# ilyakurdyukov/jpeg-quantsmooth

Measured on AMD Instinct MI355X. Metric: 8x8 blocks/s at q=3 niter=3, higher is better.
Workload: dtype f32

## Files before the change

### jpeg-quantsmooth_amd/csrc/qs_devfn.h

```cpp
#pragma once
#include <hip/hip_runtime.h>
#include <stdint.h>
#include "qs_device.h"

__device__ __forceinline__ int f2i_x86(float v) {
  return (v >= -2147483648.0f && v < 2147483648.0f) ? (int)v : (int)0x80000000;
}

__device__ __forceinline__ float round_half_away(float x) {
  float t = __builtin_truncf(x);
  float fr = __builtin_fabsf(x - t);
  return fr >= 0.5f ? t + __builtin_copysignf(1.0f, x) : t;
}

__device__ __forceinline__ void interval(int c, int div, int x1, int sh, int& orig, int& lo, int& hi) {
  int a = ((x1 * c) >> 16) + c;
  a = (int)(((uint32_t)a << sh) + 0x4000u) >> 15;
  a *= div;
  const int d0 = (div - 1) >> 1, d1 = div >> 1;
  orig = a;
  hi = a + (a < 0 ? d1 : d0);
  lo = a - (a > 0 ? d1 : d0);
}


__device__ __forceinline__ int qs_set_find(const QsPlaneSet& set, int w) {
  int lo = 0, hi = set.n - 1;
  while (lo < hi) {
    const int mid = (lo + hi + 1) >> 1;
    if (set.wave0[mid] <= w) lo = mid; else hi = mid - 1;
  }
  return lo;
}
```

### jpeg-quantsmooth_amd/csrc/qs_device.h

```cpp
#pragma once
#include <stdint.h>

#define QS_APRON_X 16
#define QS_LDS_PITCH 65
#define QS_TAB_MAX 272

enum {
  QS_DIAGONALS = 1, QS_JOINT_YUV = 2, QS_UPSAMPLE_UV = 4, QS_LOW_QUALITY = 8,
  QS_NO_REBALANCE = 16, QS_NO_REBALANCE_UV = 32, QS_TRANSCODE = 64
};

struct QsConsts {
  int32_t nat[64];
  int32_t q[64];
  int32_t qraw[64];
  int32_t x1[64];
  int32_t x2[64];
  float   range[64];
  int32_t qn[64], x1n[64], x2n[64];
  int32_t tab_size;
  int32_t pad[15];
  float   tab[64 * QS_TAB_MAX];
  int32_t rec[64][4];
};
enum {
  QS_REC_H_ANY = 1,
  QS_REC_H_SKIP4 = 2,
  QS_REC_H_EVEN = 4,
  QS_REC_V_ANY = 8,
  QS_REC_V_SKIP4 = 16,
  QS_REC_V_EVEN = 32,
  QS_REC_LDS_SHIFT = 6,
  QS_REC_NXT_SHIFT = 12,
  QS_REC_Q1 = 1 << 21
};

static inline int qs_plane_pitch(int wblk) {
  return ((wblk * 8 + QS_APRON_X + 1) + 63) & ~63;
}

#define QS_MAX_PLANES 56
struct QsPlaneRef {
  const QsConsts* cst;
  int16_t* coef;
  uint8_t* plane;
  int32_t* status;
  int32_t wblk, hblk, pitch;
  int32_t mode;
  uint8_t* plane_next;
};
enum {
  QS_PLANE_REBALANCE = 1,
  QS_PLANE_REP_TOP = 2,
  QS_PLANE_REP_BOT = 4
};
struct QsPlaneAux {
  const uint8_t* p[QS_MAX_PLANES];
};
struct QsPlaneSet {
  int32_t n, pad;
  int32_t wave0[QS_MAX_PLANES + 2];
  QsPlaneRef ref[QS_MAX_PLANES];
};
```

### jpeg-quantsmooth_amd/csrc/qs_kernels.hip

```cpp
#include <hip/hip_runtime.h>
#include <stdint.h>
#include <stdlib.h>
#include "qs_device.h"



__device__ __forceinline__ void wave_lds_sync() {
  __builtin_amdgcn_fence(__ATOMIC_RELEASE, "wavefront");
  __builtin_amdgcn_wave_barrier();
  __builtin_amdgcn_fence(__ATOMIC_ACQUIRE, "wavefront");
}

__device__ __forceinline__ uint32_t mulc(uint32_t a, int c) {
  return (uint32_t)__mul24((int)a, c);
}

__device__ __forceinline__ uint32_t lshl13_add(uint32_t x, uint32_t b) {
  uint32_t r;
  asm("v_lshl_add_u32 %0, %1, 13, %2" : "=v"(r) : "v"(x), "v"(b));
  return r;
}

__device__ __forceinline__ void idct8(uint32_t (&v)[8], uint32_t bias) {
  uint32_t z1, z2, z3, z4, z5, t0, t1, t2, t3, e0, e1, e2, e3;
  z2 = v[2]; z3 = v[6];
  z1 = mulc(z2 + z3, 4433);
  asm volatile("" : "+v"(z1));
  t2 = z1 - mulc(z3, 15137);
  t3 = z1 + mulc(z2, 6270);
  t0 = lshl13_add(v[0] + v[4], bias);
  t1 = lshl13_add(v[0] - v[4], bias);
  e0 = t0 + t3; e3 = t0 - t3; e1 = t1 + t2; e2 = t1 - t2;
  t0 = v[7]; t1 = v[5]; t2 = v[3]; t3 = v[1];
  z1 = t0 + t3; z2 = t1 + t2; z3 = t0 + t2; z4 = t1 + t3;
  z5 = mulc(z3 + z4, 9633);
  asm volatile("" : "+v"(z5));
  t0 = mulc(t0, 2446);  t1 = mulc(t1, 16819);
  t2 = mulc(t2, 25172); t3 = mulc(t3, 12299);
  z1 = mulc(z1, 7373);  z2 = mulc(z2, 20995);
  z3 = mulc(z3, 16069); z4 = mulc(z4, 3196);
  z3 = z5 - z3; z4 = z5 - z4;
  t0 += z3 - z1; t1 += z4 - z2; t2 += z3 - z2; t3 += z4 - z1;
  v[0] = e0 + t3; v[7] = e0 - t3;
  v[1] = e1 + t2; v[6] = e1 - t2;
  v[2] = e2 + t1; v[5] = e2 - t1;
  v[3] = e3 + t0; v[4] = e3 - t0;
}

__device__ __forceinline__ void idct_pass1(uint32_t (&ws)[64]) {
#pragma unroll
  for (int x = 0; x < 8; ++x) {
    uint32_t col[8];
#pragma unroll
    for (int j = 0; j < 8; ++j) col[j] = ws[j * 8 + x];
    idct8(col, 1024u);
#pragma unroll
    for (int j = 0; j < 8; ++j) ws[j * 8 + x] = (uint32_t)((int32_t)col[j] >> 11);
  }
}

__device__ __forceinline__ void idct_pass2_row(uint32_t (&row)[8], int (&out)[8]) {
  idct8(row, 257u << 17);
#pragma unroll
  for (int j = 0; j < 8; ++j) {
    int z = (int32_t)row[j];
    z = min(max(z, 0), (256 << 18) - 1);
    out[j] = z >> 18;
  }
}

#define QS_PIX_BITS 0x45000000u
__device__ __forceinline__ void idct_pass2_row_f(uint32_t (&row)[8], float (&out)[8]) {
  idct8(row, 257u << 17);
#pragma unroll
  for (int j = 0; j < 8; ++j) {
    int z = (int32_t)row[j];
    z = min(max(z, 0), (256 << 18) - 1);
    out[j] = __builtin_bit_cast(float, __builtin_amdgcn_alignbit(QS_PIX_BITS >> 14, (uint32_t)z, 18));
  }
}
__device__ __forceinline__ float pix_from_byte(uint32_t v, int n) {
  return __builtin_bit_cast(float, QS_PIX_BITS | ((v >> (8 * n)) & 0xffu));
}

__device__ __forceinline__ void
store_pixel_row(uint8_t* __restrict__ org, int pitch, int y, const int (&o)[8], int bx, int by, int wblk, int hblk,
                int rep_top, int rep_bot) {
  uint2 pk;
  pk.x = (uint32_t)o[0] | ((uint32_t)o[1] << 8) | ((uint32_t)o[2] << 16) | ((uint32_t)o[3] << 24);
  pk.y = (uint32_t)o[4] | ((uint32_t)o[5] << 8) | ((uint32_t)o[6] << 16) | ((uint32_t)o[7] << 24);
  uint8_t* rp = org + (size_t)y * pitch;
  *reinterpret_cast<uint2*>(rp) = pk;
  const bool top = (y == 0 && by == 0 && rep_top), bot = (y == 7 && by == hblk - 1 && rep_bot);
  if (bx == 0) {
    rp[-1] = (uint8_t)o[0];
    if (top) rp[-1 - pitch] = (uint8_t)o[0];
    if (bot) rp[-1 + pitch] = (uint8_t)o[0];
  }
  if (bx == wblk - 1) {
    rp[8] = (uint8_t)o[7];
    if (top) rp[8 - pitch] = (uint8_t)o[7];
    if (bot) rp[8 + pitch] = (uint8_t)o[7];
  }
  if (top) *reinterpret_cast<uint2*>(rp - pitch) = pk;
  if (bot) *reinterpret_cast<uint2*>(rp + pitch) = pk;
}

__device__ __forceinline__ void
idct_ws_to_plane(uint32_t (&ws)[64], uint8_t* __restrict__ plane, int wblk, int hblk, int pitch,
                 int rep_top, int rep_bot, int blk) {
  const int by = blk / wblk, bx = blk - by * wblk;
  idct_pass1(ws);
  uint8_t* org = plane + (size_t)(by * 8 + 1) * pitch + QS_APRON_X + bx * 8;
#pragma unroll
  for (int y = 0; y < 8; ++y) {
    uint32_t row[8]; int o[8];
#pragma unroll
    for (int j = 0; j < 8; ++j) row[j] = ws[y * 8 + j];
    idct_pass2_row(row, o);
    store_pixel_row(org, pitch, y, o, bx, by, wblk, hblk, rep_top, rep_bot);
  }
}

__device__ __forceinline__ void
idct_block_to_plane(const QsConsts* __restrict__ cst, int16_t* __restrict__ coef,
                    uint8_t* __restrict__ plane, int wblk, int hblk, int pitch,
                    int first, int rep_top, int rep_bot, int* __restrict__ status, int blk) {
  uint4* cp = reinterpret_cast<uint4*>(coef) + (size_t)blk * 8;
  uint32_t ws[64];
#pragma unroll
  for (int j = 0; j < 8; ++j) {
    uint4 v = cp[j];
    uint32_t d[4] = {v.x, v.y, v.z, v.w};
#pragma unroll
    for (int c = 0; c < 4; ++c) {
      ws[j * 8 + c * 2] = (uint32_t)(int32_t)(int16_t)(d[c] & 0xffff);
      ws[j * 8 + c * 2 + 1] = (uint32_t)((int32_t)d[c] >> 16);
    }
  }
  if (first) {
    int bad = 0;
#pragma unroll
    for (int j = 0; j < 8; ++j) {
      uint32_t d[4];
#pragma unroll
      for (int c = 0; c < 4; ++c) {
        int lo = (int32_t)ws[j * 8 + c * 2] * cst->qraw[j * 8 + c * 2];
        int hi = (int32_t)ws[j * 8 + c * 2 + 1] * cst->qraw[j * 8 + c * 2 + 1];
        bad |= ((unsigned)(lo + 0x800) > 0xfffu) | ((unsigned)(hi + 0x800) > 0xfffu);
        lo = (int16_t)lo; hi = (int16_t)hi;
        ws[j * 8 + c * 2] = (uint32_t)lo; ws[j * 8 + c * 2 + 1] = (uint32_t)hi;
        d[c] = ((uint32_t)lo & 0xffffu) | ((uint32_t)hi << 16);
      }
      cp[j] = make_uint4(d[0], d[1], d[2], d[3]);
    }
    if (bad) atomicOr(status, 1);
  }
  idct_ws_to_plane(ws, plane, wblk, hblk, pitch, rep_top, rep_bot, blk);
}

__global__ void __launch_bounds__(256)
qs_idct_plane_kernel(const QsConsts* __restrict__ cst, int16_t* __restrict__ coef,
                     uint8_t* __restrict__ plane, int wblk, int hblk, int pitch,
                     int first, int rep_top, int rep_bot, int* __restrict__ status) {
  const int blk = blockIdx.x * 256 + threadIdx.x;
  if (blk >= wblk * hblk) return;
  idct_block_to_plane(cst, coef, plane, wblk, hblk, pitch, first, rep_top, rep_bot, status, blk);
}

#include "qs_devfn.h"

__global__ void __launch_bounds__(256)
qs_idct_set_kernel(const QsPlaneSet set, int first) {
  const int w = __builtin_amdgcn_readfirstlane((int)(blockIdx.x * 4 + (threadIdx.x >> 6)));
  if (w >= set.wave0[set.n]) return;
  const int i = qs_set_find(set, w);
  const QsPlaneRef& r = set.ref[i];
  const int blk = (w - set.wave0[i]) * 64 + (threadIdx.x & 63);
  if (blk >= r.wblk * r.hblk) return;
  idct_block_to_plane(r.cst, r.coef, r.plane, r.wblk, r.hblk, r.pitch, first,
                      r.mode & QS_PLANE_REP_TOP, r.mode & QS_PLANE_REP_BOT, r.status, blk);
}



typedef int16_t __attribute__((may_alias)) lds_i16;
__device__ __forceinline__ int lds_coef(const uint32_t* col, int i) {
  const lds_i16* p = reinterpret_cast<const lds_i16*>(col + (i >> 1) * QS_LDS_PITCH) + (i & 1);
  return *p;
}
__device__ __forceinline__ void lds_set_coef(uint32_t* col, int i, int v) {
  lds_i16* p = reinterpret_cast<lds_i16*>(col + (i >> 1) * QS_LDS_PITCH) + (i & 1);
  *p = (lds_i16)v;
}

static_assert(QS_LDS_PITCH * 4 == 260, "the literal offsets below assume a 260-byte row pitch");
#define QS_LDS16_GROUP(BASE, W, N0) \
  asm volatile("ds_read_i16 %0, %16\n\tds_read_i16 %1, %16 offset:2\n\t" \
               "ds_read_i16 %2, %16 offset:260\n\tds_read_i16 %3, %16 offset:262\n\t" \
               "ds_read_i16 %4, %16 offset:520\n\tds_read_i16 %5, %16 offset:522\n\t" \
               "ds_read_i16 %6, %16 offset:780\n\tds_read_i16 %7, %16 offset:782\n\t" \
               "ds_read_i16 %8, %16 offset:1040\n\tds_read_i16 %9, %16 offset:1042\n\t" \
               "ds_read_i16 %10, %16 offset:1300\n\tds_read_i16 %11, %16 offset:1302\n\t" \
               "ds_read_i16 %12, %16 offset:1560\n\tds_read_i16 %13, %16 offset:1562\n\t" \
               "ds_read_i16 %14, %16 offset:1820\n\tds_read_i16 %15, %16 offset:1822\n\t" \
               "s_waitcnt lgkmcnt(0)" \
               : "=&v"(W[(N0) + 0]), "=&v"(W[(N0) + 1]), "=&v"(W[(N0) + 2]), "=&v"(W[(N0) + 3]), \
                 "=&v"(W[(N0) + 4]), "=&v"(W[(N0) + 5]), "=&v"(W[(N0) + 6]), "=&v"(W[(N0) + 7]), \
                 "=&v"(W[(N0) + 8]), "=&v"(W[(N0) + 9]), "=&v"(W[(N0) + 10]), "=&v"(W[(N0) + 11]), \
                 "=&v"(W[(N0) + 12]), "=&v"(W[(N0) + 13]), "=&v"(W[(N0) + 14]), "=&v"(W[(N0) + 15]) \
               : "v"(BASE) : "memory")
__device__ __forceinline__ void lds_read_block_i16(const uint32_t* col, uint32_t (&ws)[64]) {
  typedef const __attribute__((address_space(3))) uint32_t* lds_ptr;
  const uint32_t a0 = (uint32_t)(uintptr_t)(lds_ptr)col;
  const uint32_t a1 = a0 + 8 * 260, a2 = a0 + 16 * 260, a3 = a0 + 24 * 260;
  QS_LDS16_GROUP(a0, ws, 0);
  QS_LDS16_GROUP(a1, ws, 16);
  QS_LDS16_GROUP(a2, ws, 32);
  QS_LDS16_GROUP(a3, ws, 48);
}

#define QS_PIX_SCALE 0.000244140625f
#define QS_TERM_D(D, W) { \
    float u_ = __builtin_amdgcn_fmed3f(Rs - __builtin_fabsf(D), 0.0f, 1.0f); \
    float t_ = u_ * u_; \
    float x_ = (D) * t_; \
    float y_ = (W) * t_; \
    num = num + x_ * y_; \
    den = den + y_ * y_; }
#define QS_TERM(A, B, W) { float d_ = (A) - (B); QS_TERM_D(d_, W) }

typedef float qs_w16 __attribute__((ext_vector_type(16)));
typedef int qs_i4 __attribute__((ext_vector_type(4)));
#define QS_SWAIT(BUF) asm volatile("s_waitcnt lgkmcnt(0)" : "+s"(BUF) : : "memory")

#define QS_WAVES_PER_WG 4
#define QS_SMOOTH_MIN_WAVES 3
#define QS_RESIDENT_WG (256 * QS_SMOOTH_MIN_WAVES * 4 / QS_WAVES_PER_WG)
#define QS_PRIO_SLOW 3
#define QS_PRIO_TERMS 0

#define QS_TERM_OPT(COND, A, B, W) { float d_, t_; \
        asm volatile( \
          "s_cmp_lg_u32 %[c], 0\n\t" \
          "s_cbranch_scc1 1f\n\t" \
          "v_sub_f32 %[d], %[a], %[b]\n\t" \
          "v_sub_f32 %[t], %[r], |%[d]| clamp\n\t" \
          "v_mul_f32 %[t], %[t], %[t]\n\t" \
          "v_mul_f32 %[d], %[d], %[t]\n\t" \
          "v_mul_f32 %[t], %[w], %[t]\n\t" \
          "v_mul_f32 %[d], %[d], %[t]\n\t" \
          "v_add_f32 %[n], %[n], %[d]\n\t" \
          "v_mul_f32 %[d], %[t], %[t]\n\t" \
          "v_add_f32 %[e], %[e], %[d]\n" \
          "1:" \
          : [n] "+v"(num), [e] "+v"(den), [d] "=&v"(d_), [t] "=&v"(t_) \
          : [a] "v"(A), [b] "v"(B), [w] "s"(W), [r] "s"(Rs), [c] "s"(COND) : "scc"); }
#define QS_TERM_ASM(A, B, W) { float d_, t_; \
        asm volatile( \
          "v_sub_f32 %[d], %[a], %[b]\n\t" \
          "v_sub_f32 %[t], %[r], |%[d]| clamp\n\t" \
          "v_mul_f32 %[t], %[t], %[t]\n\t" \
          "v_mul_f32 %[d], %[d], %[t]\n\t" \
          "v_mul_f32 %[t], %[w], %[t]\n\t" \
          "v_mul_f32 %[d], %[d], %[t]\n\t" \
          "v_add_f32 %[n], %[n], %[d]\n\t" \
          "v_mul_f32 %[d], %[t], %[t]\n\t" \
          "v_add_f32 %[e], %[e], %[d]" \
          : [n] "+v"(num), [e] "+v"(den), [d] "=&v"(d_), [t] "=&v"(t_) \
          : [a] "v"(A), [b] "v"(B), [w] "s"(W), [r] "s"(Rs)); }

#define QS_TERM_D_ASM(D, W) { float d_, t_; \
        asm volatile( \
          "v_sub_f32 %[t], %[r], |%[a]| clamp\n\t" \
          "v_mul_f32 %[t], %[t], %[t]\n\t" \
          "v_mul_f32 %[d], %[a], %[t]\n\t" \
          "v_mul_f32 %[t], %[w], %[t]\n\t" \
          "v_mul_f32 %[d], %[d], %[t]\n\t" \
          "v_add_f32 %[n], %[n], %[d]\n\t" \
          "v_mul_f32 %[d], %[t], %[t]\n\t" \
          "v_add_f32 %[e], %[e], %[d]" \
          : [n] "+v"(num), [e] "+v"(den), [d] "=&v"(d_), [t] "=&v"(t_) \
          : [a] "v"(D), [w] "s"(W), [r] "s"(Rs)); }
#define QS_HOIST 20
#ifndef QS_HOIST_DIAG
#define QS_HOIST_DIAG 32
#endif
#ifndef QS_Q1_SKIP
#define QS_Q1_SKIP 1
#endif
#ifndef QS_STASH
#define QS_STASH 1
#endif

#define QS_SMOOTH_KERNEL_NAME qs_smooth_plane_kernel
#include "qs_smooth_kernel.inc"
#undef QS_SMOOTH_KERNEL_NAME
#define QS_SMOOTH_KERNEL_NAME qs_smooth_set_kernel
#define QS_SMOOTH_SET 1
#include "qs_smooth_kernel.inc"
#undef QS_SMOOTH_KERNEL_NAME
#undef QS_SMOOTH_SET

#define QS_DP_KERNEL_NAME qs_smooth_dp_kernel
#include "qs_smooth_dp_kernel.inc"
#undef QS_DP_KERNEL_NAME
#define QS_DP_KERNEL_NAME qs_smooth_dp_set_kernel
#define QS_DP_SET 1
#include "qs_smooth_dp_kernel.inc"
#undef QS_DP_KERNEL_NAME
#undef QS_DP_SET

__global__ void __launch_bounds__(256)
qs_clamp_kernel(int16_t* __restrict__ coef, size_t nvec) {
  size_t i = (size_t)blockIdx.x * 256 + threadIdx.x;
  const size_t stride = (size_t)gridDim.x * 256;
  uint4* p = reinterpret_cast<uint4*>(coef);
  for (; i < nvec; i += stride) {
    uint4 v = p[i];
    uint32_t d[4] = {v.x, v.y, v.z, v.w};
#pragma unroll
    for (int c = 0; c < 4; ++c) {
      int lo = (int16_t)(d[c] & 0xffff), hi = (int32_t)d[c] >> 16;
      lo = min(max(lo, -1023), 1023); hi = min(max(hi, -1023), 1023);
      d[c] = ((uint32_t)lo & 0xffffu) | ((uint32_t)hi << 16);
    }
    p[i] = make_uint4(d[0], d[1], d[2], d[3]);
  }
}

__global__ void __launch_bounds__(256)
qs_dequant_kernel(const QsConsts* __restrict__ cst, int16_t* __restrict__ coef, size_t nvec) {
  size_t i = (size_t)blockIdx.x * 256 + threadIdx.x;
  const size_t stride = (size_t)gridDim.x * 256;
  uint4* p = reinterpret_cast<uint4*>(coef);
  for (; i < nvec; i += stride) {
    uint4 v = p[i];
    uint32_t d[4] = {v.x, v.y, v.z, v.w};
    const int j = (int)(i & 7);
#pragma unroll
    for (int c = 0; c < 4; ++c) {
      int lo = (int16_t)(d[c] & 0xffff), hi = (int32_t)d[c] >> 16;
      lo *= cst->qraw[j * 8 + c * 2]; hi *= cst->qraw[j * 8 + c * 2 + 1];
      d[c] = ((uint32_t)lo & 0xffffu) | ((uint32_t)hi << 16);
    }
    p[i] = make_uint4(d[0], d[1], d[2], d[3]);
  }
}

#include "qs_launch.h"

void qs_launch_idct_plane(const QsConsts* cst, int16_t* coef, uint8_t* plane, int wblk, int hblk,
                          int first, int rep_top, int rep_bot, int* status, hipStream_t s) {
  const int nblk = wblk * hblk;
  hipLaunchKernelGGL(qs_idct_plane_kernel, dim3((nblk + 255) / 256), dim3(256), 0, s,
                     cst, coef, plane, wblk, hblk, qs_plane_pitch(wblk), first, rep_top, rep_bot, status);
}

#define QS_DP_WAVES 4
static int qs_dp_waves(int groups) {
  static const int on = [] { const char* v = getenv("QS_HIP_DP"); return v ? atoi(v) : 1; }();
  static const int lim = [] { const char* v = getenv("QS_HIP_DP_GROUPS"); return v ? atoi(v) : 768; }();
  static const int lim2 = [] { const char* v = getenv("QS_HIP_DP_GROUPS2"); return v ? atoi(v) : 1536; }();
  if (!on) return 0;
  return groups <= lim ? QS_DP_WAVES : groups <= lim2 ? 2 : 0;
}

void qs_launch_smooth_plane(const QsConsts* cst, int16_t* coef, const uint8_t* plane, uint8_t* plane_next, int rep_top, int rep_bot,
                            int wblk, int hblk, int diag, int rebalance, int final_clamp, int blk_begin, int blk_end, hipStream_t s) {
  const int n = blk_end - blk_begin;
  if (n <= 0) return;
  const int pitch = qs_plane_pitch(wblk);
  const int rep = (rep_top ? QS_PLANE_REP_TOP : 0) | (rep_bot ? QS_PLANE_REP_BOT : 0);
  if (const int nw = qs_dp_waves((n + 63) / 64)) {
    const dim3 g((n + 63) / 64), b(64 * nw);
#define QS_GO_DP(D, W) hipLaunchKernelGGL((qs_smooth_dp_kernel<D, W>), g, b, 0, s, cst, coef, plane, plane_next, rep, wblk, hblk, pitch, rebalance, final_clamp, blk_begin, blk_end)
    if (nw == 2) { if (diag) QS_GO_DP(true, 2); else QS_GO_DP(false, 2); }
    else if (diag) QS_GO_DP(true, QS_DP_WAVES); else QS_GO_DP(false, QS_DP_WAVES);
#undef QS_GO_DP
    return;
  }
  const int per_wg = 64 * QS_WAVES_PER_WG;
  const dim3 grid((n + per_wg - 1) / per_wg), block(per_wg);
#define QS_GO(K) hipLaunchKernelGGL(K, grid, block, 0, s, cst, coef, plane, plane_next, rep, wblk, hblk, pitch, rebalance, final_clamp, blk_begin, blk_end)
  if (diag) QS_GO(qs_smooth_plane_kernel<true>); else QS_GO(qs_smooth_plane_kernel<false>);
#undef QS_GO
}

void qs_launch_idct_set(const QsPlaneSet& set, int first, hipStream_t s) {
  const int nw = set.wave0[set.n];
  if (nw <= 0) return;
  hipLaunchKernelGGL(qs_idct_set_kernel, dim3((nw + 3) / 4), dim3(256), 0, s, set, first);
}

void qs_launch_smooth_set(const QsPlaneSet& set, int diag, int final_clamp, hipStream_t s) {
  const int nw = set.wave0[set.n];
  if (nw <= 0) return;
  if (const int dw = qs_dp_waves(nw)) {
    const dim3 g(nw), b(64 * dw);
#define QS_GO_DP(D, W) hipLaunchKernelGGL((qs_smooth_dp_set_kernel<D, W>), g, b, 0, s, set, final_clamp)
    if (dw == 2) { if (diag) QS_GO_DP(true, 2); else QS_GO_DP(false, 2); }
    else if (diag) QS_GO_DP(true, QS_DP_WAVES); else QS_GO_DP(false, QS_DP_WAVES);
#undef QS_GO_DP
    return;
  }
  const dim3 grid((nw + QS_WAVES_PER_WG - 1) / QS_WAVES_PER_WG), block(64 * QS_WAVES_PER_WG);
  if (diag) hipLaunchKernelGGL(qs_smooth_set_kernel<true>, grid, block, 0, s, set, final_clamp);
  else      hipLaunchKernelGGL(qs_smooth_set_kernel<false>, grid, block, 0, s, set, final_clamp);
}

void qs_launch_clamp(int16_t* coef, size_t nblk, hipStream_t s) {
  const size_t nvec = nblk * 8;
  const int grid = (int)((nvec + 255) / 256 < 8192 ? (nvec + 255) / 256 : 8192);
  hipLaunchKernelGGL(qs_clamp_kernel, dim3(grid ? grid : 1), dim3(256), 0, s, coef, nvec);
}

void qs_launch_dequant(const QsConsts* cst, int16_t* coef, size_t nblk, hipStream_t s) {
  const size_t nvec = nblk * 8;
  const int grid = (int)((nvec + 255) / 256 < 8192 ? (nvec + 255) / 256 : 8192);
  hipLaunchKernelGGL(qs_dequant_kernel, dim3(grid ? grid : 1), dim3(256), 0, s, cst, coef, nvec);
}
```

### jpeg-quantsmooth_amd/csrc/qs_smooth_kernel.inc

```
template <bool DIAG>
__global__ void __launch_bounds__(64 * QS_WAVES_PER_WG, QS_SMOOTH_MIN_WAVES)
#ifdef QS_SMOOTH_SET
QS_SMOOTH_KERNEL_NAME(const QsPlaneSet set, int final_clamp) {
  __shared__ uint32_t lds_all[QS_WAVES_PER_WG][32 * QS_LDS_PITCH];
#if QS_STASH
  __shared__ uint32_t stash_all[QS_WAVES_PER_WG][2 * 8 * 64];
#endif
  const int lane = threadIdx.x & 63, wave = threadIdx.x >> 6;
  uint32_t* lds = lds_all[wave];
  uint32_t* col = lds + lane;
  const int gw = __builtin_amdgcn_readfirstlane((int)(blockIdx.x * QS_WAVES_PER_WG + wave));
  if (gw >= set.wave0[set.n]) return;
  const int pi = qs_set_find(set, gw);
  const QsConsts* __restrict__ cst = set.ref[pi].cst;
  int16_t* __restrict__ coef = set.ref[pi].coef;
  const uint8_t* __restrict__ plane = set.ref[pi].plane;
  const int wblk = set.ref[pi].wblk, hblk = set.ref[pi].hblk, pitch = set.ref[pi].pitch;
  const int rebalance = set.ref[pi].mode & QS_PLANE_REBALANCE;
  const int nblk = wblk * hblk;
  const int base = (gw - set.wave0[pi]) * 64;
  (void)hblk;
#else
QS_SMOOTH_KERNEL_NAME(const QsConsts* __restrict__ cst, int16_t* __restrict__ coef,
                       const uint8_t* __restrict__ plane, uint8_t* __restrict__ plane_next, int rep,
                       int wblk, int hblk, int pitch,
                       int rebalance, int final_clamp, int blk_begin, int blk_end) {
  __shared__ uint32_t lds_all[QS_WAVES_PER_WG][32 * QS_LDS_PITCH];
#if QS_STASH
  __shared__ uint32_t stash_all[QS_WAVES_PER_WG][2 * 8 * 64];
#endif
  const int lane = threadIdx.x & 63, wave = threadIdx.x >> 6;
  uint32_t* lds = lds_all[wave];
  uint32_t* col = lds + lane;
  const int nblk = blk_end;
  const int base = blk_begin + (blockIdx.x * QS_WAVES_PER_WG + wave) * 64;
#endif
  if (base >= nblk) return;
  const int tail_prio = __builtin_amdgcn_readfirstlane(
      (gridDim.x > QS_RESIDENT_WG && blockIdx.x >= (gridDim.x / QS_RESIDENT_WG) * QS_RESIDENT_WG) ? 1 : 0);
  const int nvec = min(64, nblk - base) * 8;
#ifdef QS_STAGGER
  { unsigned hwid; asm volatile("s_getreg_b32 %0, hwreg(HW_REG_HW_ID)" : "=s"(hwid)); if (hwid & 1u) __builtin_amdgcn_s_sleep(QS_STAGGER); }
#endif

  uint4* gsrc = reinterpret_cast<uint4*>(coef) + (size_t)base * 8;
  {
    const int m0 = (lane & 7) * 4;
#pragma unroll
    for (int j = 0; j < 8; ++j) {
      const int idx = j * 64 + lane;
      uint4 v = make_uint4(0, 0, 0, 0);
      if (idx < nvec) v = gsrc[idx];
      uint32_t* dst = lds + m0 * QS_LDS_PITCH + (j * 8 + (lane >> 3));
      dst[0] = v.x; dst[QS_LDS_PITCH] = v.y; dst[2 * QS_LDS_PITCH] = v.z; dst[3 * QS_LDS_PITCH] = v.w;
    }
  }

  const int blk = min(base + lane, nblk - 1);
  const int by = blk / wblk, bx = blk - by * wblk;
  const uint8_t* org = plane + (size_t)(by * 8 + 1) * pitch + QS_APRON_X + bx * 8;
  uint32_t edge[8];
  {
    const uint2 t = *reinterpret_cast<const uint2*>(org - pitch);
    const uint2 b = *reinterpret_cast<const uint2*>(org + (size_t)8 * pitch);
    edge[0] = t.x; edge[1] = t.y; edge[2] = b.x; edge[3] = b.y;
    uint32_t l[8], r[8];
#pragma unroll
    for (int y = 0; y < 8; ++y) {
      l[y] = org[(ptrdiff_t)y * pitch - 1];
      r[y] = org[(ptrdiff_t)y * pitch + 8];
    }
    edge[4] = l[0] | (l[1] << 8) | (l[2] << 16) | (l[3] << 24);
    edge[5] = l[4] | (l[5] << 8) | (l[6] << 16) | (l[7] << 24);
    edge[6] = r[0] | (r[1] << 8) | (r[2] << 16) | (r[3] << 24);
    edge[7] = r[4] | (r[5] << 8) | (r[6] << 16) | (r[7] << 24);
  }
  wave_lds_sync();

  constexpr int TS = DIAG ? 272 : 160;
  float px[64];
  float bd[32];
  constexpr int NH = DIAG ? QS_HOIST_DIAG : QS_HOIST;
  float hd[NH];

  int kfirst = 63;
#if QS_STASH
  int stash_hi = 0;
#endif
  uint32_t chg = 0;
  long long reb_m0 = 0, reb_m1 = 0;
  const float* tabp = cst->tab;
  const int32_t* recp = &cst->rec[0][0];
  qs_w16 WA, WB;
  qs_i4 REC;
  qs_i4 RECN;
  asm volatile("s_load_dwordx4 %0, %2, %3\n\ts_load_dwordx16 %1, %4, %5\n\ts_waitcnt lgkmcnt(0)"
               : "=&s"(REC), "=&s"(WA) : "s"(recp), "s"(63u * 16u), "s"(tabp), "s"((uint32_t)63 * (TS * 4)) : "memory");
  RECN = REC;

#pragma unroll 1
  for (int g = 0; g < 14; ++g) {
    __builtin_amdgcn_s_setprio(QS_PRIO_SLOW);
    if (g == 0 || __builtin_amdgcn_ballot_w64(chg != 0) != 0) {
      chg = 0;
      uint32_t ws[64];
      lds_read_block_i16(col, ws);
#if QS_STASH
      {
        uint32_t* stash = stash_all[wave] + lane;
#pragma unroll
        for (int x = 0; x < 8; ++x) {
          uint32_t c[8];
          const bool low = x <= 1, high = x >= 6;
          const int slot = (x == 0 || x == 7) ? 0 : 1;
          bool reuse = false, store = false;
          if (low) { reuse = g >= 1 && g <= 7 - x; store = g == 0; }
          if (high) {
            const int fin = 15 - x;
            const bool have = (stash_hi >> (x - 6)) & 1;
            reuse = g >= fin && have; store = g >= fin && !have;
          }
          if ((low || high) && reuse) {
#pragma unroll
            for (int j = 0; j < 8; ++j) c[j] = stash[(slot * 8 + j) * 64];
          } else {
#pragma unroll
            for (int j = 0; j < 8; ++j) c[j] = ws[j * 8 + x];
            idct8(c, 1024u);
#pragma unroll
            for (int j = 0; j < 8; ++j) c[j] = (uint32_t)((int32_t)c[j] >> 11);
            if ((low || high) && store) {
#pragma unroll
              for (int j = 0; j < 8; ++j) stash[(slot * 8 + j) * 64] = c[j];
              if (high) stash_hi |= 1 << (x - 6);
            }
          }
#pragma unroll
          for (int j = 0; j < 8; ++j) ws[j * 8 + x] = c[j];
        }
      }
#else
      idct_pass1(ws);
#endif
#pragma unroll
      for (int y = 0; y < 8; ++y) {
        uint32_t row[8]; float o[8];
#pragma unroll
        for (int j = 0; j < 8; ++j) row[j] = ws[y * 8 + j];
        idct_pass2_row_f(row, o);
#pragma unroll
        for (int j = 0; j < 8; ++j) px[y * 8 + j] = o[j];
      }
#pragma unroll
      for (int e = 0; e < 8; ++e) asm volatile("" : "+v"(edge[e]));
#pragma unroll
      for (int x = 0; x < 8; ++x) {
        bd[x]      = px[x]         - pix_from_byte(edge[0 + (x >> 2)], x & 3);
        bd[8 + x]  = px[56 + x]    - pix_from_byte(edge[2 + (x >> 2)], x & 3);
        bd[16 + x] = px[x * 8]     - pix_from_byte(edge[4 + (x >> 2)], x & 3);
        bd[24 + x] = px[x * 8 + 7] - pix_from_byte(edge[6 + (x >> 2)], x & 3);
      }
#pragma unroll
      for (int t = 0; t < NH; ++t) hd[t] = px[(t / 7) * 8 + t % 7] - px[(t / 7) * 8 + t % 7 + 1];
    }
    const int len = min(g + 1, 15 - g);
    const int klast = max(kfirst - len + 1, 1);
#pragma unroll 1
    for (int k = kfirst; k >= klast; --k) {
#pragma unroll
      for (int p = 0; p < 64; ++p) asm volatile("" : "+v"(px[p]));
      const int md = REC[3];
      const int x2k = (REC[0] >> 16) & 31, qk = REC[1] & 0xffff, x1k = REC[1] >> 16;
      const uint32_t lds_off = ((uint32_t)md >> QS_REC_LDS_SHIFT) & 0x3fffu;
      int rs_bits = REC[2];
      asm volatile("" : "+s"(rs_bits));
      const float Rs = __builtin_bit_cast(float, rs_bits);
      const uint32_t kb = (uint32_t)k * (TS * 4);
      const uint32_t kb_nxt = kb - (uint32_t)(TS * 4);
      const uint32_t kb_s = (uint32_t)__builtin_amdgcn_readfirstlane((int)kb);
      const uint32_t kb_nxt_s = (uint32_t)__builtin_amdgcn_readfirstlane((int)kb_nxt);
      const uint32_t next_first = kb_nxt + (((uint32_t)md >> QS_REC_NXT_SHIFT) & 0x100u);
      const uint32_t after_V = DIAG ? kb + 640u : next_first;
      const uint32_t after_B = (md & QS_REC_V_ANY) ? kb + 384u : after_V;
#if QS_Q1_SKIP
      if (__builtin_expect(md & QS_REC_Q1, 0)) {
        {
          const int c0 = *reinterpret_cast<lds_i16*>(reinterpret_cast<char*>(col) + lds_off);
          reb_m0 += (long long)(c0 * c0);
          reb_m1 += (long long)(c0 * c0);
        }
        asm volatile("s_load_dwordx16 %0, %2, %3\n\ts_load_dwordx4 %1, %4, %5\n\ts_waitcnt lgkmcnt(0)"
                     : "=&s"(WA), "=&s"(RECN)
                     : "s"(tabp), "s"((uint32_t)__builtin_amdgcn_readfirstlane((int)next_first)), "s"(recp),
                       "s"((uint32_t)(k - 1) * 16u) : "memory");
        REC = RECN;
      } else
#endif
      {
      float num = 0.0f, den = 0.0f;
      asm volatile("s_setprio %c1\n\ts_cmp_eq_u32 %0, 0\n\ts_cbranch_scc1 1f\n\ts_setprio %c2\n1:"
                   : : "s"(tail_prio), "i"(QS_PRIO_TERMS), "i"(QS_PRIO_TERMS + 1) : "scc");

#define QS_ROW_D(W, Y) { \
        _Pragma("unroll") for (int x = 0; x < 7; ++x) { \
          QS_TERM(px[(Y) * 8 + x], px[(Y) * 8 + x + 9], W[x]) \
          QS_TERM(px[(Y) * 8 + x + 1], px[(Y) * 8 + x + 8], W[8 + x]) } }
#define QS_EDGE16(W, J0) { \
        _Pragma("unroll") for (int j = 0; j < 16; ++j) QS_TERM_D(bd[(J0) + j], W[j]) }
#define QS_HOISTED_TERM(T, WT) else if ((T) < NH) QS_TERM_D_ASM(hd[(T) % NH], WT)
#define QS_ROWS_H_M(W, Y0, MODE) { \
        _Pragma("unroll") for (int yy = 0; yy < 2; ++yy) \
        _Pragma("unroll") for (int x = 0; x < 7; ++x) { \
          if (((MODE) == 2 && (x & 1)) || ((MODE) == 1 && x == 3)) {} \
          QS_HOISTED_TERM(((Y0) + yy) * 7 + x, W[yy * 8 + x]) \
          else QS_TERM_ASM(px[((Y0) + yy) * 8 + x], px[((Y0) + yy) * 8 + x + 1], W[yy * 8 + x]) } }
#define QS_ROWS_V_M(W, Y0, NY, MODE) { \
        _Pragma("unroll") for (int yy = 0; yy < (NY); ++yy) \
        _Pragma("unroll") for (int x = 0; x < 8; ++x) { \
          if (((MODE) == 2 && (((Y0) + yy) & 1)) || ((MODE) == 1 && (Y0) + yy == 3)) {} \
          else QS_TERM_ASM(px[((Y0) + yy) * 8 + x], px[((Y0) + yy) * 8 + x + 8], W[yy * 8 + x]) } }

      const uint32_t rec_next = (uint32_t)(k - 1) * 16u;
#define QS_ISSUE(NXT, BYTEOFF) \
      asm volatile("s_load_dwordx16 %0, %3, %4" : "=&s"(NXT), "+v"(num), "+v"(den) \
                   : "s"(tabp), "s"((uint32_t)__builtin_amdgcn_readfirstlane((int)(BYTEOFF))) : "memory")
#define QS_ISSUE_K(NXT, IMM) \
      asm volatile("s_load_dwordx16 %0, %3, %4 offset:%c5" : "=&s"(NXT), "+v"(num), "+v"(den) \
                   : "s"(tabp), "s"(kb_s), "i"(IMM) : "memory")
#define QS_LAND(NXT) asm volatile("s_waitcnt lgkmcnt(0)" : "+s"(NXT), "+v"(num), "+v"(den) : : "memory")
#define QS_ISSUE_R(NXT, BYTEOFF) \
      asm volatile("s_load_dwordx16 %0, %4, %5\n\ts_load_dwordx4 %1, %6, %7" : "=&s"(NXT), "=&s"(RECN), "+v"(num), "+v"(den) \
                   : "s"(tabp), "s"((uint32_t)__builtin_amdgcn_readfirstlane((int)(BYTEOFF))), "s"(recp), "s"(rec_next) : "memory")
#define QS_LAND_R(NXT) asm volatile("s_waitcnt lgkmcnt(0)" : "+s"(NXT), "+s"(RECN), "+v"(num), "+v"(den) : : "memory")
#define QS_T4(O) "s_load_dword %1, %4, %5 offset:" #O "\n\ts_load_dword %1, %4, %5 offset:" #O "+0x40\n\ts_load_dword %1, %4, %5 offset:" #O "+0x80\n\ts_load_dword %1, %4, %5 offset:" #O "+0xc0\n\t"
#define QS_ISSUE_T(NXT, IMM) \
      uint32_t touch; \
      if (DIAG) asm volatile("s_load_dwordx16 %0, %4, %6 offset:%c7\n\t" QS_T4(0x0) QS_T4(0x100) QS_T4(0x200) QS_T4(0x300) "s_load_dword %1, %4, %5 offset:0x400" \
                   : "=&s"(NXT), "=&s"(touch), "+v"(num), "+v"(den) \
                   : "s"(tabp), "s"(kb_nxt_s), "s"(kb_s), "i"(IMM) : "memory"); \
      else      asm volatile("s_load_dwordx16 %0, %4, %6 offset:%c7\n\t" QS_T4(0x0) QS_T4(0x100) "s_load_dword %1, %4, %5 offset:0x200\n\ts_load_dword %1, %4, %5 offset:0x240" \
                   : "=&s"(NXT), "=&s"(touch), "+v"(num), "+v"(den) \
                   : "s"(tabp), "s"(kb_nxt_s), "s"(kb_s), "i"(IMM) : "memory")
#define QS_LAND_T(NXT) asm volatile("s_waitcnt lgkmcnt(0)" : "+s"(NXT), "+s"(touch), "+v"(num), "+v"(den) : : "memory")
#define QS_H_SECTION(MODE) { \
        QS_ISSUE_K(WB, 64);  QS_ROWS_H_M(WA, 0, MODE) QS_LAND(WB); \
        QS_ISSUE_K(WA, 128); QS_ROWS_H_M(WB, 2, MODE) QS_LAND(WA); \
        QS_ISSUE_K(WB, 192); QS_ROWS_H_M(WA, 4, MODE) QS_LAND(WB); \
        QS_ISSUE_K(WA, 256); QS_ROWS_H_M(WB, 6, MODE) QS_LAND(WA); }
      if (md & QS_REC_H_ANY) {
        if (md & QS_REC_H_SKIP4) QS_H_SECTION(2)
        else if (md & QS_REC_H_EVEN) QS_H_SECTION(1)
        else QS_H_SECTION(0)
      }
      QS_ISSUE_T(WB, 320); QS_EDGE16(WA, 0) QS_LAND_T(WB);
      if (!DIAG && !(md & QS_REC_V_ANY)) { QS_ISSUE_R(WA, after_B); QS_EDGE16(WB, 16) QS_LAND_R(WA); }
      else                   { QS_ISSUE(WA, after_B);   QS_EDGE16(WB, 16) QS_LAND(WA); }
#define QS_V_SECTION(MODE) { \
        QS_ISSUE_K(WB, 448); QS_ROWS_V_M(WA, 0, 2, MODE) QS_LAND(WB); \
        QS_ISSUE_K(WA, 512); QS_ROWS_V_M(WB, 2, 2, MODE) QS_LAND(WA); \
        QS_ISSUE_K(WB, 576); QS_ROWS_V_M(WA, 4, 2, MODE) QS_LAND(WB); \
        if (!DIAG) { QS_ISSUE_R(WA, after_V); QS_ROWS_V_M(WB, 6, 1, MODE) QS_LAND_R(WA); } \
        else       { QS_ISSUE(WA, after_V);   QS_ROWS_V_M(WB, 6, 1, MODE) QS_LAND(WA); } }
      if (md & QS_REC_V_ANY) {
        if (md & QS_REC_V_SKIP4) QS_V_SECTION(2)
        else if (md & QS_REC_V_EVEN) QS_V_SECTION(1)
        else QS_V_SECTION(0)
      }
      if (DIAG) {
        QS_ISSUE_K(WB, 704);  QS_ROW_D(WA, 0) QS_LAND(WB);
        QS_ISSUE_K(WA, 768);  QS_ROW_D(WB, 1) QS_LAND(WA);
        QS_ISSUE_K(WB, 832);  QS_ROW_D(WA, 2) QS_LAND(WB);
        QS_ISSUE_K(WA, 896);  QS_ROW_D(WB, 3) QS_LAND(WA);
        QS_ISSUE_K(WB, 960);  QS_ROW_D(WA, 4) QS_LAND(WB);
        QS_ISSUE_K(WA, 1024); QS_ROW_D(WB, 5) QS_LAND(WA);
        QS_ISSUE_R(WB, next_first); QS_ROW_D(WA, 6) QS_LAND_R(WB);
        WA = WB;
      }
#undef QS_ROWS_H_M
#undef QS_HOISTED_TERM
#undef QS_ROWS_V_M
#undef QS_H_SECTION
#undef QS_V_SECTION
#undef QS_ISSUE
#undef QS_ISSUE_K
#undef QS_LAND
#undef QS_ISSUE_R
#undef QS_LAND_R
#undef QS_ISSUE_T
#undef QS_LAND_T
#undef QS_T4

      __builtin_amdgcn_s_setprio(QS_PRIO_SLOW);
      lds_i16* const cptr = reinterpret_cast<lds_i16*>(reinterpret_cast<char*>(col) + lds_off);
      const int c0 = *cptr;
      const int r = f2i_x86(round_half_away((num / den) * 4096.0f));
      {
        int orig, lo, hi;
        interval(c0, qk, x1k, x2k, orig, lo, hi);
        int v = (int)((uint32_t)c0 - (uint32_t)r);
        v = min(max(v, lo), hi);
        *cptr = (lds_i16)v;
        chg |= (uint32_t)(v ^ c0);
        if (rebalance) {
          reb_m0 += (long long)(v * orig);
          reb_m1 += (long long)(orig * orig);
        }
      }
      REC = RECN;
      }
    }
    kfirst = klast - 1;
  }
  QS_SWAIT(WA);

  if (rebalance) {
    const long long m0 = reb_m0, m1 = reb_m1;
    if (m1 > m0) {
      const int mul = (int)(((m1 << 13) + (m0 >> 1)) / m0);
#pragma unroll 9
      for (int n = 1; n < 64; ++n) {
        const int c = lds_coef(col, n);
        int orig, lo, hi;
        interval(c, cst->qn[n], cst->x1n[n], cst->x2n[n], orig, lo, hi);
        int v = (c * mul + 0x1000) >> 13;
        v = min(max(v, lo), hi);
        lds_set_coef(col, n, v);
      }
    }
  }
  wave_lds_sync();

  {
    int lane2 = lane;
    asm volatile("" : "+v"(lane2));
    const int lane = lane2;
    const int m0 = (lane & 7) * 4;
#pragma unroll
    for (int j = 0; j < 8; ++j) {
      const int idx = j * 64 + lane;
      const uint32_t* s = lds + m0 * QS_LDS_PITCH + (j * 8 + (lane >> 3));
      uint32_t d[4] = {s[0], s[QS_LDS_PITCH], s[2 * QS_LDS_PITCH], s[3 * QS_LDS_PITCH]};
      if (final_clamp) {
#pragma unroll
        for (int c = 0; c < 4; ++c) {
          int lo = (int16_t)(d[c] & 0xffff), hi = (int32_t)d[c] >> 16;
          lo = min(max(lo, -1023), 1023); hi = min(max(hi, -1023), 1023);
          d[c] = ((uint32_t)lo & 0xffffu) | ((uint32_t)hi << 16);
        }
      }
      if (idx < nvec) gsrc[idx] = make_uint4(d[0], d[1], d[2], d[3]);
    }
  }

#ifdef QS_SMOOTH_SET
  int pi2 = pi;
  asm volatile("" : "+s"(pi2));
  uint8_t* __restrict__ plane_next = set.ref[pi2].plane_next;
  const int rep = set.ref[pi2].mode, wblk2 = set.ref[pi2].wblk, hblk2 = set.ref[pi2].hblk, pitch2 = set.ref[pi2].pitch;
#else
  const int wblk2 = wblk, hblk2 = hblk, pitch2 = pitch;
#endif
  if (plane_next) {
    uint32_t ws[64];
    lds_read_block_i16(col, ws);
    if (base + lane < nblk)
      idct_ws_to_plane(ws, plane_next, wblk2, hblk2, pitch2, rep & QS_PLANE_REP_TOP, rep & QS_PLANE_REP_BOT, base + lane);
  }
}

#undef QS_ROW_D
#undef QS_EDGE16
```

### jpeg-quantsmooth_amd/csrc/qs_tables.cpp

```cpp
#include <stdarg.h>
#include <math.h>
#include <mutex>

#include "qs_xfer.h"

static thread_local char g_err[512] = "";

int qs_fail(int code, const char* fmt, ...) {
  va_list ap; va_start(ap, fmt);
  vsnprintf(g_err, sizeof(g_err), fmt, ap);
  va_end(ap);
  return code;
}


extern "C" const char* qs_hip_last_error(void) { return g_err; }

extern "C" int qs_hip_device_count(void) {
  int n = 0;
  if (hipGetDeviceCount(&n) != hipSuccess) { (void)hipGetLastError(); return 0; }
  return n;
}

extern "C" size_t qs_hip_consts_bytes(void) { return sizeof(QsConsts); }
extern "C" size_t qs_hip_plane_pitch(int wblk) { return (size_t)qs_plane_pitch(wblk); }
extern "C" size_t qs_hip_plane_bytes(int wblk, int hblk) {
  return (size_t)qs_plane_pitch(wblk) * ((size_t)hblk * 8 + 2) + 64;
}
extern "C" size_t qs_hip_plane_row_offset(int wblk, int y) {
  return (size_t)qs_plane_pitch(wblk) * (size_t)(y + 1);
}
extern "C" void qs_hip_free(void* p) { if (p && !qsx::pinned_return(p)) free(p); }


static const unsigned char kZigzag[64] = {
  0, 1, 8, 16, 9, 2, 3, 10, 17, 24, 32, 25, 18, 11, 4, 5,
  12, 19, 26, 33, 40, 48, 41, 34, 27, 20, 13, 6, 7, 14, 21, 28,
  35, 42, 49, 56, 57, 50, 43, 36, 29, 22, 15, 23, 30, 37, 44, 51,
  58, 59, 52, 45, 38, 31, 39, 46, 53, 60, 61, 54, 47, 55, 62, 63
};

static void idct8f(const float* in, int is, float* out, int os, bool scale) {
  float z1, z2, z3, z4, z5, t0, t1, t2, t3, t4, t5, t6, t7;
  z2 = in[2 * is]; z3 = in[6 * is];
  z1 = (z2 + z3) * 0.541196100f;
  t2 = z1 - z3 * 1.847759065f;
  t3 = z1 + z2 * 0.765366865f;
  z2 = in[0]; z3 = in[4 * is];
  t0 = z2 + z3; t1 = z2 - z3;
  t4 = t0 + t3; t7 = t0 - t3; t5 = t1 + t2; t6 = t1 - t2;
  t0 = in[7 * is]; t1 = in[5 * is]; t2 = in[3 * is]; t3 = in[is];
  z1 = t0 + t3; z2 = t1 + t2; z3 = t0 + t2; z4 = t1 + t3;
  z5 = (z3 + z4) * 1.175875602f;
  t0 = t0 * 0.298631336f; t1 = t1 * 2.053119869f;
  t2 = t2 * 3.072711026f; t3 = t3 * 1.501321110f;
  z1 = z1 * 0.899976223f; z2 = z2 * 2.562915447f;
  z3 = z3 * 1.961570560f; z4 = z4 * 0.390180644f;
  z3 = z3 - z5; t0 = t0 - (z1 + z3); t2 = t2 - (z2 + z3);
  z4 = z4 - z5; t1 = t1 - (z2 + z4); t3 = t3 - (z1 + z4);
  float r[8] = { t4 + t3, t5 + t2, t6 + t1, t7 + t0, t7 - t0, t6 - t1, t5 - t2, t4 - t3 };
  for (int j = 0; j < 8; ++j) out[j * os] = scale ? r[j] * 0.125f : r[j];
}

static void impulse_response(int i, float T[64]) {
  float in[64], ws[64];
  memset(in, 0, sizeof(in)); in[i] = 1.0f;
  for (int x = 0; x < 8; ++x) idct8f(in + x, 8, ws + x, 8, false);
  for (int y = 0; y < 8; ++y) idct8f(ws + y * 8, 1, T + y * 8, 1, true);
}

struct WeightTables {
  float tab[2][64 * QS_TAB_MAX];
  int status[2];
  char msg[2][160];
};

static void build_tables(WeightTables& W, int diag) {
  const int ts = diag ? 272 : 160;
  const float b = diag ? 4.0f : 2.0f;
  float* tab = W.tab[diag];
  memset(tab, 0, sizeof(W.tab[diag]));
  W.status[diag] = QS_HIP_OK;
  for (int k = 0; k < 64; ++k) {
    const int i = kZigzag[k];
    float T[64], *w = tab + (size_t)k * ts;
    impulse_response(i, T);
    for (int y = 0; y < 8; ++y) for (int x = 0; x < 8; ++x) {
      const int p = y * 8 + x;
      w[p] = x < 7 ? T[p] - T[p + 1] : 0.0f;
      w[96 + p] = y < 7 ? T[p] - T[p + 8] : 0.0f;
    }
    for (int x = 0; x < 8; ++x) {
      w[64 + x] = T[x] * b; w[72 + x] = T[56 + x] * b;
      w[80 + x] = T[8 * x] * b; w[88 + x] = T[8 * x + 7] * b;
    }
    if (diag)
      for (int y = 0; y < 7; ++y) for (int x = 0; x < 8; ++x) {
        const int p = y * 8 + x;
        w[160 + 16 * y + x] = x < 7 ? T[p] - T[p + 9] : 0.0f;
        w[168 + 16 * y + x] = x < 7 ? T[p + 1] - T[p + 8] : 0.0f;
      }
  }
  for (int k = 1; k < 64; ++k) {
    const int i = kZigzag[k], u = i & 7, v = i >> 3;
    const float* w = tab + (size_t)k * ts;
    for (int y = 0; y < 8; ++y) for (int x = 0; x < 7; ++x)
      if (u && ((x + 1) * u) % 8 == 0 && w[y * 8 + x] != 0.0f) {
        W.status[diag] = QS_HIP_EINVAL;
        snprintf(W.msg[diag], sizeof(W.msg[diag]), "weight table: expected exact zero at k=%d h(%d,%d)", k, y, x);
      }
    for (int y = 0; y < 7; ++y) for (int x = 0; x < 8; ++x)
      if (v && ((y + 1) * v) % 8 == 0 && w[96 + y * 8 + x] != 0.0f) {
        W.status[diag] = QS_HIP_EINVAL;
        snprintf(W.msg[diag], sizeof(W.msg[diag]), "weight table: expected exact zero at k=%d v(%d,%d)", k, y, x);
      }
  }
  for (size_t j = 0; j < (size_t)64 * ts; ++j) {
    const float a = tab[j] < 0 ? -tab[j] : tab[j];
    if (a != 0.0f && a < 2.3283064e-10f ) {
      W.status[diag] = QS_HIP_EINVAL;
      snprintf(W.msg[diag], sizeof(W.msg[diag]), "weight table entry %g too small for the scaled evaluation", (double)a);
    }
  }
}

static const WeightTables& weight_tables() {
  static WeightTables* W = [] {
    WeightTables* w = new WeightTables;
    build_tables(*w, 0);
    build_tables(*w, 1);
    return w;
  }();
  return *W;
}

extern "C" int qs_hip_consts_build(void* host_out, const uint16_t quant[64], int flags) {
  if (!host_out || !quant) return qs_fail(QS_HIP_EINVAL, "qs_hip_consts_build: null argument");
  QsConsts* c = static_cast<QsConsts*>(host_out);
  const int diag = (flags & QS_DIAGONALS) != 0;
  const int ts = diag ? 272 : 160;
  const WeightTables& W = weight_tables();
  if (W.status[diag] != QS_HIP_OK) return qs_fail(W.status[diag], "%s", W.msg[diag]);
  memset(c, 0, offsetof(QsConsts, tab));
  c->tab_size = ts;
  int qn[64], x1n[64], x2n[64];
  for (int i = 0; i < 64; ++i) {
    unsigned q = quant[i] ? quant[i] : 1u, n = 0, t = q;
    while (t > 1) { t >>= 1; ++n; }
    unsigned x1 = ((0x10000u << n) + q - 1) / q;
    if (n) x1 |= x1 >> 16;
    const int sh = 15 - (int)n;
    qn[i] = (int)q; x1n[i] = (int16_t)(uint16_t)x1; x2n[i] = sh;
    c->qraw[i] = quant[i];
    c->qn[i] = qn[i]; c->x1n[i] = x1n[i]; c->x2n[i] = x2n[i];
  }
  for (int k = 0; k < 64; ++k) {
    const int i = kZigzag[k];
    c->nat[k] = i; c->q[k] = qn[i]; c->x1[k] = x1n[i]; c->x2[k] = x2n[i];
    c->range[k] = (float)(qn[i] * 2) * 0.000244140625f;
  }
  for (int k = 0; k < 64; ++k) {
    const int kn = k > 1 ? k - 1 : 1;
    c->rec[k][0] = c->nat[k] | (c->nat[kn] << 8) | (c->x2[k] << 16);
    c->rec[k][1] = (int32_t)(((uint32_t)c->q[k] & 0xffffu) | ((uint32_t)c->x1[k] << 16));
    memcpy(&c->rec[k][2], &c->range[k], sizeof(float));
    {
      const int i = c->nat[k], u = i & 7, v = i >> 3, i_nxt = c->nat[kn];
      int m = 0;
      if (u) m |= QS_REC_H_ANY;
      if (u == 4) m |= QS_REC_H_SKIP4;
      if (!(u & 1)) m |= QS_REC_H_EVEN;
      if (v) m |= QS_REC_V_ANY;
      if (v == 4) m |= QS_REC_V_SKIP4;
      if (!(v & 1)) m |= QS_REC_V_EVEN;
      m |= ((i >> 1) * QS_LDS_PITCH * 4 + (i & 1) * 2) << QS_REC_LDS_SHIFT;
      if (!(i_nxt & 7)) m |= 0x100 << QS_REC_NXT_SHIFT;
      if (c->q[k] == 1) m |= QS_REC_Q1;
      c->rec[k][3] = m;
    }
  }
  memcpy(c->tab, W.tab[diag], sizeof(c->tab));
  return QS_HIP_OK;
}
```

Before: 273.6 million.

## Use fast reciprocal quotient, 32-bit rebalance sums, and per-lane refresh skipping

The exact float division plus round-half-away is replaced by a reciprocal multiply with rint and a conservative error check. If any lane fails the check, the whole wave falls back to the exact path. Rebalance accumulators use 32-bit mul24 sums when a ballot shows all coefficients and quant values are small, otherwise manual 64-bit carry adds, and the rebalance loop uses mul24 when the multiplier fits in 24 bits. In early iterations, lanes with no changes also skip the block refresh, trading extra divergence and mode-selection logic for fewer 64-bit and division operations.

```diff
diff --git a/jpeg-quantsmooth_amd/csrc/qs_devfn.h b/jpeg-quantsmooth_amd/csrc/qs_devfn.h
--- a/jpeg-quantsmooth_amd/csrc/qs_devfn.h
+++ b/jpeg-quantsmooth_amd/csrc/qs_devfn.h
@@ -2,6 +2,10 @@
 #include <hip/hip_runtime.h>
 #include <stdint.h>
 #include "qs_device.h"
+
+#ifndef QS_FAST_QUOT
+#define QS_FAST_QUOT 1
+#endif
 
 __device__ __forceinline__ int f2i_x86(float v) {
   return (v >= -2147483648.0f && v < 2147483648.0f) ? (int)v : (int)0x80000000;
@@ -11,6 +15,51 @@
   float t = __builtin_truncf(x);
   float fr = __builtin_fabsf(x - t);
   return fr >= 0.5f ? t + __builtin_copysignf(1.0f, x) : t;
+}
+
+__device__ __forceinline__ int qs_quot_exact(float num, float den) {
+  return f2i_x86(round_half_away((num / den) * 4096.0f));
+}
+
+__device__ __forceinline__ int qs_quot_fast(float num, float den, bool& ok) {
+  const float z = (num * __builtin_amdgcn_rcpf(den)) * 4096.0f;
+  const float n = __builtin_rintf(z);
+  ok = (__float_as_uint(den) - 0x00800000u) < (0x7e000000u - 0x00800000u) &&
+       __builtin_fmaf(__builtin_fabsf(z), 0x1p-21f, __builtin_fabsf(z - n)) < 0.5f;
+  return (int)n;
+}
+
+__device__ __forceinline__ int qs_quot(float num, float den) {
+#if QS_FAST_QUOT
+  bool ok;
+  int r = qs_quot_fast(num, den, ok);
+  if (__builtin_amdgcn_ballot_w64(!ok) != 0) r = qs_quot_exact(num, den);
+  return r;
+#else
+  return qs_quot_exact(num, den);
+#endif
+}
+
+struct QsRebSums { uint32_t lo0, hi0, lo1, hi1; };
+__device__ __forceinline__ void qs_reb_add64(uint32_t& lo, uint32_t& hi, int p) {
+  const uint32_t l = lo + (uint32_t)p;
+  hi += (uint32_t)(p >> 31) + (l < (uint32_t)p ? 1u : 0u);
+  lo = l;
+}
+__device__ __forceinline__ void qs_reb_add(QsRebSums& s, int mode, int v, int orig) {
+  if (mode == 1) {
+    s.lo0 += (uint32_t)__mul24(v, orig);
+    s.lo1 += (uint32_t)__mul24(orig, orig);
+  } else {
+    qs_reb_add64(s.lo0, s.hi0, v * orig);
+    qs_reb_add64(s.lo1, s.hi1, orig * orig);
+  }
+}
+__device__ __forceinline__ long long qs_reb_m0(const QsRebSums& s, int mode) {
+  return mode == 1 ? (long long)(int32_t)s.lo0 : (long long)(((uint64_t)s.hi0 << 32) | s.lo0);
+}
+__device__ __forceinline__ long long qs_reb_m1(const QsRebSums& s, int mode) {
+  return mode == 1 ? (long long)(int32_t)s.lo1 : (long long)(((uint64_t)s.hi1 << 32) | s.lo1);
 }
 
 __device__ __forceinline__ void interval(int c, int div, int x1, int sh, int& orig, int& lo, int& hi) {
diff --git a/jpeg-quantsmooth_amd/csrc/qs_device.h b/jpeg-quantsmooth_amd/csrc/qs_device.h
--- a/jpeg-quantsmooth_amd/csrc/qs_device.h
+++ b/jpeg-quantsmooth_amd/csrc/qs_device.h
@@ -19,7 +19,8 @@
   float   range[64];
   int32_t qn[64], x1n[64], x2n[64];
   int32_t tab_size;
-  int32_t pad[15];
+  int32_t qmax;
+  int32_t pad[14];
   float   tab[64 * QS_TAB_MAX];
   int32_t rec[64][4];
 };
diff --git a/jpeg-quantsmooth_amd/csrc/qs_kernels.hip b/jpeg-quantsmooth_amd/csrc/qs_kernels.hip
--- a/jpeg-quantsmooth_amd/csrc/qs_kernels.hip
+++ b/jpeg-quantsmooth_amd/csrc/qs_kernels.hip
@@ -292,6 +292,12 @@
 #ifndef QS_STASH
 #define QS_STASH 1
 #endif
+#ifndef QS_REB32
+#define QS_REB32 1
+#endif
+#ifndef QS_REFRESH_LANES
+#define QS_REFRESH_LANES 1
+#endif
 
 #define QS_SMOOTH_KERNEL_NAME qs_smooth_plane_kernel
 #include "qs_smooth_kernel.inc"
diff --git a/jpeg-quantsmooth_amd/csrc/qs_smooth_kernel.inc b/jpeg-quantsmooth_amd/csrc/qs_smooth_kernel.inc
--- a/jpeg-quantsmooth_amd/csrc/qs_smooth_kernel.inc
+++ b/jpeg-quantsmooth_amd/csrc/qs_smooth_kernel.inc
@@ -44,6 +44,7 @@
 #endif
 
   uint4* gsrc = reinterpret_cast<uint4*>(coef) + (size_t)base * 8;
+  uint32_t wide = 0;
   {
     const int m0 = (lane & 7) * 4;
 #pragma unroll
@@ -51,6 +52,9 @@
       const int idx = j * 64 + lane;
       uint4 v = make_uint4(0, 0, 0, 0);
       if (idx < nvec) v = gsrc[idx];
+#if QS_REB32
+      wide |= (v.x ^ (v.x << 1)) | (v.y ^ (v.y << 1)) | (v.z ^ (v.z << 1)) | (v.w ^ (v.w << 1));
+#endif
       uint32_t* dst = lds + m0 * QS_LDS_PITCH + (j * 8 + (lane >> 3));
       dst[0] = v.x; dst[QS_LDS_PITCH] = v.y; dst[2 * QS_LDS_PITCH] = v.z; dst[3 * QS_LDS_PITCH] = v.w;
     }
@@ -84,11 +88,21 @@
   float hd[NH];
 
   int kfirst = 63;
+#if QS_REFRESH_LANES
+#ifdef QS_SMOOTH_SET
+  constexpr bool lanes = true;
+#else
+  constexpr bool lanes = !DIAG;
+#endif
+#endif
 #if QS_STASH
   int stash_hi = 0;
 #endif
   uint32_t chg = 0;
-  long long reb_m0 = 0, reb_m1 = 0;
+  QsRebSums reb = {0, 0, 0, 0};
+  const int reb_mode = __builtin_amdgcn_readfirstlane(
+      !rebalance ? 0 : (QS_REB32 && cst->qmax <= 1024 && __builtin_amdgcn_ballot_w64((wide & 0xe000e000u) != 0) == 0) ? 1 : 2);
+  (void)wide;
   const float* tabp = cst->tab;
   const int32_t* recp = &cst->rec[0][0];
   qs_w16 WA, WB;
@@ -101,7 +115,11 @@
 #pragma unroll 1
   for (int g = 0; g < 14; ++g) {
     __builtin_amdgcn_s_setprio(QS_PRIO_SLOW);
-    if (g == 0 || __builtin_amdgcn_ballot_w64(chg != 0) != 0) {
+    if (g == 0 || __builtin_amdgcn_ballot_w64(chg != 0) != 0)
+#if QS_REFRESH_LANES
+    if (!lanes || g == 0 || g >= 8 || chg != 0)
+#endif
+    {
       chg = 0;
       uint32_t ws[64];
       lds_read_block_i16(col, ws);
@@ -186,8 +204,7 @@
       if (__builtin_expect(md & QS_REC_Q1, 0)) {
         {
           const int c0 = *reinterpret_cast<lds_i16*>(reinterpret_cast<char*>(col) + lds_off);
-          reb_m0 += (long long)(c0 * c0);
-          reb_m1 += (long long)(c0 * c0);
+          qs_reb_add(reb, reb_mode, c0, c0);
         }
         asm volatile("s_load_dwordx16 %0, %2, %3\n\ts_load_dwordx4 %1, %4, %5\n\ts_waitcnt lgkmcnt(0)"
                      : "=&s"(WA), "=&s"(RECN)
@@ -293,7 +310,7 @@
       __builtin_amdgcn_s_setprio(QS_PRIO_SLOW);
       lds_i16* const cptr = reinterpret_cast<lds_i16*>(reinterpret_cast<char*>(col) + lds_off);
       const int c0 = *cptr;
-      const int r = f2i_x86(round_half_away((num / den) * 4096.0f));
+      const int r = qs_quot(num, den);
       {
         int orig, lo, hi;
         interval(c0, qk, x1k, x2k, orig, lo, hi);
@@ -301,10 +318,7 @@
         v = min(max(v, lo), hi);
         *cptr = (lds_i16)v;
         chg |= (uint32_t)(v ^ c0);
-        if (rebalance) {
-          reb_m0 += (long long)(v * orig);
-          reb_m1 += (long long)(orig * orig);
-        }
+        if (reb_mode) qs_reb_add(reb, reb_mode, v, orig);
       }
       REC = RECN;
       }
@@ -313,19 +327,22 @@
   }
   QS_SWAIT(WA);
 
-  if (rebalance) {
-    const long long m0 = reb_m0, m1 = reb_m1;
+  if (reb_mode) {
+    const long long m0 = qs_reb_m0(reb, reb_mode), m1 = qs_reb_m1(reb, reb_mode);
     if (m1 > m0) {
       const int mul = (int)(((m1 << 13) + (m0 >> 1)) / m0);
-#pragma unroll 9
-      for (int n = 1; n < 64; ++n) {
-        const int c = lds_coef(col, n);
-        int orig, lo, hi;
-        interval(c, cst->qn[n], cst->x1n[n], cst->x2n[n], orig, lo, hi);
-        int v = (c * mul + 0x1000) >> 13;
-        v = min(max(v, lo), hi);
-        lds_set_coef(col, n, v);
-      }
+#define QS_REB_LOOP(CMUL) \
+      _Pragma("unroll 9") for (int n = 1; n < 64; ++n) { \
+        const int c = lds_coef(col, n); \
+        int orig, lo, hi; \
+        interval(c, (int)(uint16_t)cst->qn[n], (int)(int16_t)cst->x1n[n], cst->x2n[n], orig, lo, hi); \
+        int v = ((CMUL) + 0x1000) >> 13; \
+        v = min(max(v, lo), hi); \
+        lds_set_coef(col, n, v); \
+      }
+      if (QS_REB32 && __builtin_amdgcn_ballot_w64(mul < -(1 << 23) || mul >= (1 << 23)) == 0) QS_REB_LOOP(__mul24(c, mul))
+      else QS_REB_LOOP(c * mul)
+#undef QS_REB_LOOP
     }
   }
   wave_lds_sync();
diff --git a/jpeg-quantsmooth_amd/csrc/qs_tables.cpp b/jpeg-quantsmooth_amd/csrc/qs_tables.cpp
--- a/jpeg-quantsmooth_amd/csrc/qs_tables.cpp
+++ b/jpeg-quantsmooth_amd/csrc/qs_tables.cpp
@@ -153,6 +153,7 @@
     qn[i] = (int)q; x1n[i] = (int16_t)(uint16_t)x1; x2n[i] = sh;
     c->qraw[i] = quant[i];
     c->qn[i] = qn[i]; c->x1n[i] = x1n[i]; c->x2n[i] = x2n[i];
+    if (qn[i] > c->qmax) c->qmax = qn[i];
   }
   for (int k = 0; k < 64; ++k) {
     const int i = kZigzag[k];
```

Result: no change. 272.3 million (median of 2 runs) (-0.5%).
